# Koukyosyumei/MyZKP

Hardware: AMD Instinct MI355X
Metric: G1 MSM pairs/sec + NTT elems/sec at 2^20 and 2^24; bit-exact vs CPU (higher is better)
Workload: dtype u32x9 (29-bit limbs, 254-bit Montgomery); 1 GPU; KZG commit = BN254 G1 Pippenger MSM of 2^20 (scalar, point) pairs per GPU against a device-resident SRS (commit_kzg, kzg.rs:57-59); 17-bit signed windows (library default at this size), 15 window tables built once at upload; N GPUs = one MSM of N*2^20 pairs (BASELINE configs[2]/[3]); pairs_per_gpu=1048576, seed=332211571536, window_bits=17

## Files before the change

### myzkp_amd/csrc/mzk_msm.hip

```cpp
#include <stdlib.h>
#include <type_traits>
#include "mzk_common.h"
#include "mzk_ec.h"
#include "mzk_coop.h"
#include "mzk_row.h"
#include "mzk_glv.h"
#include "mzk_affine_wave.h"

namespace mzk {

static const MsmKnobs& msm_knobs() {
  static const MsmKnobs k = [] {
    const MsmKnobs d;
    return MsmKnobs{tune_int("MZK_GLV_C", d.glv_c), tune_int("MZK_SMALL_SCAN", d.small_scan), tune_int("MZK_SCAN_MAX_LOG", d.scan_max_log),
                    tune_int("MZK_ACC_PREFETCH", d.acc_prefetch), tune_int("MZK_ACC_SEG", d.acc_seg), tune_int("MZK_COARSE_LOG_20", d.coarse_log_20),
                    tune_int("MZK_COARSE_LOG_17", d.coarse_log_17), tune_int("MZK_PER_FINE", d.per_fine), tune_int("MZK_SORT_SCAN_FREE", d.sort_scan_free),
                    tune_int("MZK_COMBINE_WIDE_MIN_LOG", d.combine_wide_min_log)};
  }();
  return k;
}

int msm_generic_window_bits(size_t n) { return choose_shape_glv(n ? n : 1, msm_knobs().glv_c).c; }

__device__ __forceinline__ void load_words8(const u32* __restrict__ g, u32* w) {
  const uint4* p4 = reinterpret_cast<const uint4*>(g);
  uint4 a = p4[0], b = p4[1];
  w[0] = a.x; w[1] = a.y; w[2] = a.z; w[3] = a.w; w[4] = b.x; w[5] = b.y; w[6] = b.z; w[7] = b.w;
}
__device__ __forceinline__ void store_words8(u32* __restrict__ g, const u32* w) {
  uint4* p4 = reinterpret_cast<uint4*>(g);
  p4[0] = make_uint4(w[0], w[1], w[2], w[3]);
  p4[1] = make_uint4(w[4], w[5], w[6], w[7]);
}
__device__ __forceinline__ Xyzz xyzz_gload(const u32* __restrict__ g, size_t idx) {
  u32 w[32];
#pragma unroll
  for (int q = 0; q < 4; q++) load_words8(g + idx * 32 + 8 * q, w + 8 * q);
  return xyzz_load(w);
}
__device__ __forceinline__ void xyzz_gstore(u32* __restrict__ g, size_t idx, const Xyzz& p) {
  u32 w[32];
  xyzz_store(p, w);
#pragma unroll
  for (int q = 0; q < 4; q++) store_words8(g + idx * 32 + 8 * q, w + 8 * q);
}

static_assert(SLOT_WORDS == 4 * FqParams::L, "a slot is the four raw coordinates");
__device__ __forceinline__ void xyzz_gstore_raw(u32* __restrict__ g, size_t idx, const Xyzz& p) {
  u32 w[SLOT_WORDS];
  const bool inf = xyzz_is_inf(p);
#pragma unroll
  for (int i = 0; i < FqParams::L; i++) {
    w[i] = inf ? 0u : p.X.l[i]; w[9 + i] = inf ? 0u : p.Y.l[i]; w[18 + i] = inf ? 0u : p.ZZ.l[i]; w[27 + i] = inf ? 0u : p.ZZZ.l[i];
  }
  uint4* p4 = reinterpret_cast<uint4*>(g + idx * SLOT_WORDS);
#pragma unroll
  for (int q = 0; q < SLOT_WORDS / 4; q++) p4[q] = make_uint4(w[4 * q], w[4 * q + 1], w[4 * q + 2], w[4 * q + 3]);
}
__device__ __forceinline__ Xyzz xyzz_gload_raw(const u32* __restrict__ g, size_t idx) {
  u32 w[SLOT_WORDS];
  const uint4* p4 = reinterpret_cast<const uint4*>(g + idx * SLOT_WORDS);
#pragma unroll
  for (int q = 0; q < SLOT_WORDS / 4; q++) { const uint4 v = p4[q]; w[4 * q] = v.x; w[4 * q + 1] = v.y; w[4 * q + 2] = v.z; w[4 * q + 3] = v.w; }
  Xyzz p;
#pragma unroll
  for (int i = 0; i < FqParams::L; i++) { p.X.l[i] = w[i]; p.Y.l[i] = w[9 + i]; p.ZZ.l[i] = w[18 + i]; p.ZZZ.l[i] = w[27 + i]; }
  return p;
}
__device__ __forceinline__ Xyzz xyzz_gload_raw_quad(const u32* __restrict__ g, size_t idx, int lane) {
  Fq mine;
  const u32* src = g + idx * SLOT_WORDS + 9 * lane;
#pragma unroll
  for (int i = 0; i < FqParams::L; i++) mine.l[i] = src[i];
  Xyzz p;
  p.X = quad_bcast<0>(mine);
  p.Y = quad_bcast<1>(mine);
  p.ZZ = quad_bcast<2>(mine);
  p.ZZZ = quad_bcast<3>(mine);
  return p;
}

__global__ void k_prepare_points(const u32* __restrict__ in, u32* __restrict__ out, size_t n, u32* __restrict__ phi_out) {
  const size_t i = (size_t)blockIdx.x * blockDim.x + threadIdx.x;
  if (i >= n) return;
  u32 w[16];
  load_words8(in + i * 16, w);
  load_words8(in + i * 16 + 8, w + 8);
  Affine a;
  const bool inf = affine_words_is_inf(w);
  if (!inf) {
    a = affine_load_plain(w);
    affine_store_mont(a, w);
  }
  store_words8(out + i * 16, w);
  store_words8(out + i * 16 + 8, w + 8);
  if (phi_out) {
    if (!inf) {
      Fq beta;
// ... 614 lines not shown
#pragma unroll
    for (int k = 0; k < STAGE_PER_LANE; k++) rk[k] = (chunk + tid + k * SORT2_THREADS < cend) ? counter_inc_agg(cnt, REC::fine(r[k], fmask, fb)) : 0u;
    __syncthreads();
    u32 local = 0;
    for (int q = 0; q < per; q++) { const int f = tid * per + q; if (f < F) local += cnt[f]; }
    u32 run = block_excl_scan<SORT2_THREADS>(local, scan, nullptr);
    for (int q = 0; q < per; q++) { const int f = tid * per + q; if (f < F) { lpre[f] = run; run += cnt[f]; } }
    __syncthreads();
#pragma unroll
    for (int k = 0; k < STAGE_PER_LANE; k++) {
      if (chunk + tid + k * SORT2_THREADS < cend) {
        const u32 fk = REC::fine(r[k], fmask, fb);
        const u32 pos = lpre[fk] + rk[k];
        spay[pos] = REC::payload(r[k], fb);
        skey[pos] = (unsigned short)fk;
      }
    }
    __syncthreads();
    const u32 m = cend - chunk;
    for (u32 j = tid; j < m; j += SORT2_THREADS) {
      const u32 f = skey[j];
      entries[gbase[f] + (j - lpre[f])] = spay[j];
    }
    __syncthreads();
    for (int f = tid; f < F; f += SORT2_THREADS) gbase[f] += cnt[f];
    __syncthreads();
  }
}

__global__ __launch_bounds__(256) void k_scan_local(const u32* __restrict__ in, u32* __restrict__ out, u32* __restrict__ block_sums, size_t n) {
  __shared__ u32 sh[256];
  const size_t base = (size_t)blockIdx.x * SCAN_BLOCK + (size_t)threadIdx.x * SCAN_ITEMS;
  u32 v[SCAN_ITEMS], sum = 0;
#pragma unroll
  for (int k = 0; k < SCAN_ITEMS; k++) {
    v[k] = (base + k < n) ? in[base + k] : 0u;
    sum += v[k];
  }
  u32 block_total;
  u32 excl = block_excl_scan<256>(sum, sh, &block_total);
  if (threadIdx.x == 255) block_sums[blockIdx.x] = block_total;
#pragma unroll
  for (int k = 0; k < SCAN_ITEMS; k++) {
    if (base + k < n) out[base + k] = excl;
    excl += v[k];
  }
}
__global__ __launch_bounds__(256) void k_scan_finish(u32* __restrict__ offsets, const u32* __restrict__ block_sums, size_t nblocks, size_t n) {
  __shared__ u32 part[4];
  static_assert(SCAN_BLOCK % 256 == 0, "one block index per workgroup");
  const size_t i = (size_t)blockIdx.x * blockDim.x + threadIdx.x;
  const size_t first = (size_t)blockIdx.x * blockDim.x;
  const bool total_wg = first >= n;
  const size_t blk = total_wg ? nblocks : first / SCAN_BLOCK;
  u32 acc = 0;
  for (size_t j = threadIdx.x; j < blk; j += 256) acc += block_sums[j];
#pragma unroll
  for (int d = 32; d >= 1; d >>= 1) acc += (u32)__shfl_xor((int)acc, d, 64);
  if ((threadIdx.x & 63) == 0) part[threadIdx.x >> 6] = acc;
  __syncthreads();
  const u32 pre = part[0] + part[1] + part[2] + part[3];
  if (total_wg) { if (threadIdx.x == 0) offsets[n] = pre; }
  else if (i < n) offsets[i] = offsets[i] + pre;
}

__global__ __launch_bounds__(256) void k_scan_add(u32* __restrict__ offsets, const u32* __restrict__ prefix, size_t nblocks, size_t n) {
  const size_t i = (size_t)blockIdx.x * blockDim.x + threadIdx.x;
  if (i < n) offsets[i] += prefix[i / SCAN_BLOCK];
  else if (i == n) offsets[n] = prefix[nblocks];
}
static int launch_exclusive_scan(const u32* in, u32* out, size_t n, u32* scratch, hipStream_t s) {
  const size_t sb = (n + SCAN_BLOCK - 1) / SCAN_BLOCK;
  hipLaunchKernelGGL(k_scan_local, dim3((unsigned)sb), dim3(256), 0, s, in, out, scratch, n);
  if (sb <= SCAN_DIRECT_BLOCKS) {
    hipLaunchKernelGGL(k_scan_finish, dim3((unsigned)((n + 255) / 256 + 1)), dim3(256), 0, s, out, (const u32*)scratch, sb, n);
  } else {
    MZK_TRY(launch_exclusive_scan((const u32*)scratch, scratch, sb, scratch + sb + 2, s));
    hipLaunchKernelGGL(k_scan_add, dim3((unsigned)(n / 256 + 1)), dim3(256), 0, s, out, (const u32*)scratch, sb, n);
  }
  MZK_HIP(hipGetLastError());
  return MZK_OK;
}

constexpr u32 MANY_SENTINEL = 0xffffffffu;
constexpr u32 SEG_MIN = 8;
__device__ __forceinline__ u32 segment_length(u32 seg_host, u32 t_max, u32 total_entries) {
  if (t_max == 0) return seg_host;
  const u32 v = (total_entries + t_max - 1) / t_max;
  return v < SEG_MIN ? SEG_MIN : v;
}
template <bool PREFETCH, bool SENT = false>
__global__ __launch_bounds__(256) void k_seg_accumulate(const u32* __restrict__ points_mont, const u32* __restrict__ offsets,
                                                         const u32* __restrict__ entries, u32* __restrict__ slots, size_t nbuckets,
                                                         u32 seg_host, u32 t_max) {
  const size_t t = (size_t)blockIdx.x * blockDim.x + threadIdx.x;
  const u32 total_entries = offsets[nbuckets];
  const u32 seg = segment_length(seg_host, t_max, total_entries);
  const u64 e0w = (u64)t * seg;
  if (e0w >= total_entries) return;
  const u32 e0 = (u32)e0w;
  const u32 e1 = (e0w + seg < total_entries) ? e0 + seg : total_entries;
  size_t lo = 0, hi = nbuckets;
  while (hi - lo > 1) {
    const size_t mid = (lo + hi) >> 1;
    if (offsets[mid] <= e0) lo = mid; else hi = mid;
  }
  size_t b = lo;
  u32 bend = offsets[b + 1];
  Xyzz acc = xyzz_inf();
  u32 ent_next = entries[e0];
  u32 wn[16];
  if (PREFETCH) {
    const size_t idx = ent_next & 0x7fffffffu;
    load_words8(points_mont + idx * 16, wn);
    load_words8(points_mont + idx * 16 + 8, wn + 8);
  }
  for (u32 e = e0; e < e1; e++) {
    const u32 ent = ent_next;
    u32 w[16];
    if (PREFETCH) {
#pragma unroll
      for (int k = 0; k < 16; k++) w[k] = wn[k];
    } else {
      const size_t idx = (SENT && ent == MANY_SENTINEL) ? 0 : (ent & 0x7fffffffu);
      load_words8(points_mont + idx * 16, w);
      load_words8(points_mont + idx * 16 + 8, w + 8);
    }
    if (e + 1 < e1) {
      ent_next = entries[e + 1];
      if (PREFETCH) {
        const size_t idx = ent_next & 0x7fffffffu;
        load_words8(points_mont + idx * 16, wn);
        load_words8(points_mont + idx * 16 + 8, wn + 8);
      }
    }
    if (e >= bend) {
      xyzz_gstore_raw(slots, t + b, acc);
      acc = xyzz_inf();
      do { b++; bend = offsets[b + 1]; } while (e >= bend);
    }
    if (affine_words_is_inf(w)) continue;
    if (SENT && ent == MANY_SENTINEL) continue;
    acc = xyzz_madd_signed_with<FeAsm>(acc, affine_load_mont(w), (ent >> 31) != 0);
  }
  xyzz_gstore_raw(slots, t + b, acc);
}
constexpr u32 HEAVY_SLOTS_SORT1 = 16;
__device__ __forceinline__ u32 bucket_end(const u32* __restrict__ offsets, const u32* __restrict__ tails, int lg_nb, size_t b) {
  if (tails && (b & (((size_t)1 << lg_nb) - 1)) == (((size_t)1 << lg_nb) - 1)) return tails[b >> lg_nb];
  return offsets[b + 1];
}
__device__ __forceinline__ bool defer_heavy(size_t b, size_t s0, size_t s1, u32 o1, u32* __restrict__ heavy, bool leader, u32 threshold = HEAVY_SLOTS) {
  if (s1 - s0 + 1 <= threshold) return false;
  if (leader) { const u32 i = atomicAdd(&heavy[0], 1u); heavy[HEAVY_HDR + 2 * i] = (u32)b; heavy[HEAVY_HDR + 2 * i + 1] = o1; }
  return true;
}
__global__ __launch_bounds__(128) void k_seg_combine_wide(const u32* __restrict__ slots, const u32* __restrict__ offsets,
                                                           u32* __restrict__ buckets, size_t nbuckets, u32 seg_host, u32* __restrict__ heavy, u32 t_max) {
  const size_t b = (size_t)blockIdx.x * blockDim.x + threadIdx.x;
  if (b >= nbuckets) return;
  const u32 seg = segment_length(seg_host, t_max, offsets[nbuckets]);
  if (b == 0) heavy[1] = seg;
  const u32 o0 = offsets[b], o1 = offsets[b + 1];
  Xyzz acc = xyzz_inf();
  if (o1 > o0) {
    const size_t s0 = (size_t)(o0 / seg) + b, s1 = (size_t)((o1 - 1) / seg) + b;
    if (defer_heavy(b, s0, s1, o1, heavy, true)) return;
    for (size_t sl = s0; sl <= s1; sl++) acc = xyzz_add_with<FeAsm>(acc, xyzz_gload_raw(slots, sl));
  }
  xyzz_gstore(buckets, b, acc);
}
__global__ __launch_bounds__(128) void k_seg_combine(const u32* __restrict__ slots, const u32* __restrict__ offsets, u32* __restrict__ buckets,
                                                      size_t nbuckets, u32 seg_host, u32* __restrict__ heavy, const u32* __restrict__ tails, int lg_nb, u32 t_max) {
  const size_t tid = (size_t)blockIdx.x * blockDim.x + threadIdx.x;
  const size_t b = tid / 4;
  const int lane = (int)(tid & 3);
  if (b >= nbuckets) return;
  const u32 seg = segment_length(seg_host, t_max, offsets[nbuckets]);
  if (tid == 0) heavy[1] = seg;
  const u32 o0 = offsets[b], o1 = bucket_end(offsets, tails, lg_nb, b);
  Xyzz acc = xyzz_inf();
  if (o1 > o0) {
    const size_t s0 = (size_t)(o0 / seg) + b, s1 = (size_t)((o1 - 1) / seg) + b;
    if (defer_heavy(b, s0, s1, o1, heavy, lane == 0, tails ? HEAVY_SLOTS_SORT1 : HEAVY_SLOTS)) return;
    acc = xyzz_gload_raw_quad(slots, s0, lane);
    for (size_t sl = s0 + 1; sl <= s1; sl++) acc = xyzz_add_quad(acc, xyzz_gload_raw_quad(slots, sl, lane), lane);
  }
  xyzz_gstore_quad(buckets, b, acc, lane);
}
constexpr int HEAVY_THREADS = 256;
constexpr int HEAVY_QUADS = HEAVY_THREADS / 4;
__device__ __forceinline__ void heavy_tree(u32* sh, const Xyzz& acc, int quad, int lane) {
  xyzz_gstore_quad(sh, quad, acc, lane);
  __syncthreads();
  for (int off = HEAVY_QUADS / 2; off >= 1; off >>= 1) {
    if (quad < off) {
      const Xyzz x = xyzz_gload_quad(sh, quad, lane), y = xyzz_gload_quad(sh, quad + off, lane);
      xyzz_gstore_quad(sh, quad, xyzz_add_quad(x, y, lane), lane);
    }
    __syncthreads();
  }
}
__global__ __launch_bounds__(HEAVY_THREADS) void k_seg_combine_heavy(const u32* __restrict__ slots, const u32* __restrict__ offsets,
                                                                      u32* __restrict__ buckets, u32* __restrict__ heavy, size_t max_heavy) {
  __shared__ __attribute__((aligned(16))) u32 sh[HEAVY_QUADS * 32];
  __shared__ u32 last_arrival;
  const u32 count = heavy[0];
  if (count == 0) return;
  const u32 seg = heavy[1];
  const int lane = threadIdx.x & 3, quad = threadIdx.x >> 2;
  const u32* list = heavy + HEAVY_HDR;
  if (2 * count > gridDim.x) {
    for (u32 h = blockIdx.x; h < count; h += gridDim.x) {
      const size_t b = list[2 * h];
      const u32 o0 = offsets[b], o1 = list[2 * h + 1];
      const size_t s0 = (size_t)(o0 / seg) + b, s1 = (size_t)((o1 - 1) / seg) + b;
      Xyzz acc = xyzz_inf();
      for (size_t sl = s0 + quad; sl <= s1; sl += HEAVY_QUADS) acc = xyzz_add_quad(acc, xyzz_gload_raw_quad(slots, sl, lane), lane);
      heavy_tree(sh, acc, quad, lane);
      if (quad == 0) xyzz_gstore_quad(buckets, b, xyzz_gload_quad(sh, 0, lane), lane);
      __syncthreads();
    }
    return;
  }
  const u32 G = gridDim.x / count;
  const u32 h = blockIdx.x / G, part = blockIdx.x % G;
  if (h >= count) return;
  u32* scratch = heavy + heavy_list_words(max_heavy);
// ... 398 lines not shown
      *slots = nullptr, *wghist = nullptr, *wsum = nullptr;
  const struct { WsSlot slot; size_t bytes; u32** p; size_t words; } req[] = {
      {WS_MSM_POINTS, P.ws.points, &pm, 0}, {WS_MSM_COUNTS, P.ws.counts, &counts, 0}, {WS_MSM_OFFSETS, P.ws.offsets, &offsets, P.NBtot + 1},
      {WS_MSM_CURSOR, P.ws.cursor, &ranks, 0}, {WS_MSM_ENTRIES, P.ws.entries, &entries, P.alloc.E}, {WS_MSM_SCAN, P.ws.scan, &scan, 0},
      {WS_MSM_BUCKETS, P.ws.buckets, &buckets, P.NB * 32}, {WS_MSM_SLOTS, P.ws.slots, &slots, P.slot_region_words},
      {WS_MSM_WGHIST, P.ws.wghist, &wghist, 0}, {WS_MSM_OUT, P.ws.out, &wsum, 0}};
  for (const auto& r : req)
    if (r.bytes) { MZK_TRY(ws_get(r.slot, r.bytes, (void**)r.p)); *r.p += (cc ? cc->k : 0) * r.words; }
  const u32* pts = (pm ? pm : (const u32*)d_points) + i0 * 16;
  bool prepared = false;
  auto prepare = [&]() -> int {
    if (prepared) return MZK_OK;
    prepared = true;
    if (points_ready) MZK_TRY((*points_ready)());
    if (!pm) return MZK_OK;
    prof_begin(s, MZK_PH_MSM_PREPARE);
    MZK_TRY(msm_prepare_points((const u32*)d_points + i0 * 16, n, pm + i0 * 16, pm + (n_shape + i0) * 16, s));
    prof_end(s, MZK_PH_MSM_PREPARE);
    return MZK_OK;
  };
  if (P.path == MsmPath::SmallScan) {
    MZK_TRY(prepare());
    prof_begin(s, MZK_PH_MSM_ACCUMULATE);
#define MZK_SCAN_CASE(C) case C: hipLaunchKernelGGL((k_small_accumulate_scan<256, C>), dim3((unsigned)P.NB), dim3(256), 0, s, (const u32*)d_scalars, n, P.L.table_stride, pts, buckets); break;
    switch (P.L.c) { MZK_SCAN_CASE(8) MZK_SCAN_CASE(10) MZK_SCAN_CASE(11) MZK_SCAN_CASE(12) MZK_SCAN_CASE(13) }
#undef MZK_SCAN_CASE
    prof_end(s, MZK_PH_MSM_ACCUMULATE);
  } else if (P.path == MsmPath::SmallSort) {
    MZK_TRY(prepare());
    prof_begin(s, MZK_PH_MSM_SORT);
    hipLaunchKernelGGL(k_small_sort, dim3(1), dim3(SMALL_SORT_THREADS), (P.NB + SMALL_SORT_THREADS) * 4, s, (const u32*)d_scalars, n, P.L, (int)P.NB, offsets, entries);
    prof_end(s, MZK_PH_MSM_SORT);
    prof_begin(s, MZK_PH_MSM_ACCUMULATE);
    if (P.small_wide)
      hipLaunchKernelGGL(k_small_accumulate<256>, dim3((unsigned)P.NB), dim3(256), 0, s, pts, (const u32*)offsets, (const u32*)entries, buckets);
    else
      hipLaunchKernelGGL(k_small_accumulate<64>, dim3((unsigned)P.NB), dim3(64), 0, s, pts, (const u32*)offsets, (const u32*)entries, buckets);
    prof_end(s, MZK_PH_MSM_ACCUMULATE);
  } else {
    u32* heavy = slots + P.nslots * SLOT_WORDS;
    prof_begin(s, MZK_PH_MSM_SORT);
    MZK_HIP(hipMemsetAsync(heavy, 0, (size_t)HEAVY_HDR * 4, s));
    if (P.path == MsmPath::TwoLevel) {
      u32* finehist = wghist + P.alloc.n_coarse + 1;
      const SortBufs sb{(const u32*)d_scalars, wghist, ranks, finehist, scan + scan_scratch_words(P.alloc.n_coarse) + 2, offsets, entries,
                        P.coarse_free ? heavy + SORT_CTR_AT : nullptr, P.coarse_free ? heavy + SORT_CTR_AT + SORT_CTR_BINS : nullptr,
                        P.coarse_free ? finehist + P.alloc.n_fine + 1 : nullptr, P.fine_free ? counts : nullptr, P.fine_free ? counts + P.NBtot : nullptr};
#define MZK_CCOUNT(C, CLOG) hipLaunchKernelGGL((k_coarse_count<C, CLOG>), dim3(P.nwg), dim3(SORT2_THREADS), 0, s, (const u32*)d_scalars, n, P.L, P.key_shift, wghist, \
                                               P.nwg, sb.bin_tot, sb.bucket_tot, P.fine_free ? 2 * P.NBtot : (size_t)0)
      if (P.coarse_c == 20 && P.cl == 10) MZK_CCOUNT(20, 10);
      else if (P.coarse_c == 17 && P.cl == 9) MZK_CCOUNT(17, 9);
      else if (P.cl == 10) MZK_CCOUNT(0, 10);
      else if (P.coarse_c == 20) MZK_CCOUNT(20, COARSE_LOG);
      else if (P.coarse_c == 17) MZK_CCOUNT(17, COARSE_LOG);
      else if (P.coarse_c == 16) MZK_CCOUNT(16, COARSE_LOG);
      else MZK_CCOUNT(0, COARSE_LOG);
#undef MZK_CCOUNT
      if (!P.coarse_free) MZK_TRY(launch_exclusive_scan((const u32*)wghist, wghist, P.own.n_coarse, scan, s));
      MZK_TRY(P.compact ? sort_records<Rec4>(P, sb, s) : sort_records<Rec8>(P, sb, s));
    } else if (P.path == MsmPath::LdsOnePass) {
      const size_t lds = P.NB * 4;
      bool& lds_attr_set = ctx().attr_done[ATTR_DIGITS_LDS];
      if (!lds_attr_set) {
        MZK_HIP(hipFuncSetAttribute((const void*)k_digits_count_lds, hipFuncAttributeMaxDynamicSharedMemorySize, 160 * 1024));
        MZK_HIP(hipFuncSetAttribute((const void*)k_digits_scatter_lds, hipFuncAttributeMaxDynamicSharedMemorySize, 160 * 1024));
        lds_attr_set = true;
      }
      hipLaunchKernelGGL(k_digits_count_lds, dim3(P.nwg), dim3(LDS_SORT_THREADS), lds, s, (const u32*)d_scalars, n, P.per_wg, P.L, wghist, ranks);
      hipLaunchKernelGGL(k_wg_hist_prefix, dim3((unsigned)((P.NB + 255) / 256)), dim3(256), 0, s, wghist, P.nwg, (int)P.NB, counts);
      MZK_TRY(launch_exclusive_scan((const u32*)counts, offsets, P.NB, scan, s));
      hipLaunchKernelGGL(k_digits_scatter_lds, dim3(P.nwg), dim3(LDS_SORT_THREADS), lds, s, (const u32*)d_scalars, n, P.per_wg, P.L, (const u32*)offsets,
                         (const u32*)wghist, (const u32*)ranks, entries);
    } else {
      const unsigned nblk = (unsigned)((n + 255) / 256);
      MZK_HIP(hipMemsetAsync(counts, 0, P.NB * 4, s));
      hipLaunchKernelGGL(k_digits_count, dim3(nblk), dim3(256), 0, s, (const u32*)d_scalars, n, P.L, counts, ranks);
      MZK_TRY(launch_exclusive_scan((const u32*)counts, offsets, P.NB, scan, s));
      hipLaunchKernelGGL(k_digits_scatter, dim3(nblk), dim3(256), 0, s, (const u32*)d_scalars, n, P.L, offsets, ranks, entries);
    }
    MZK_HIP(hipGetLastError());
    prof_end(s, MZK_PH_MSM_SORT);
    MZK_TRY(prepare());
    prof_begin(s, MZK_PH_MSM_ACCUMULATE);
#ifdef MZK_TUNING
    if (P.prefetch)
      hipLaunchKernelGGL(k_seg_accumulate<true>, dim3((unsigned)((P.T + 255) / 256)), dim3(256), 0, s, pts, offsets, entries, slots, P.NB, P.seg, P.t_max);
    else
#endif
      hipLaunchKernelGGL(k_seg_accumulate<false>, dim3((unsigned)((P.T + 255) / 256)), dim3(256), 0, s, pts, offsets, entries, slots, P.NB, P.seg, P.t_max);
    prof_end(s, MZK_PH_MSM_ACCUMULATE);
    prof_begin(s, MZK_PH_MSM_SEG_COMBINE);
    if (P.combine_wide)
      hipLaunchKernelGGL(k_seg_combine_wide, dim3((unsigned)((P.NB + 127) / 128)), dim3(128), 0, s, slots, offsets, buckets, P.NB, P.seg, heavy, P.t_max);
    else
      hipLaunchKernelGGL(k_seg_combine, dim3((unsigned)((4 * P.NB + 127) / 128)), dim3(128), 0, s, slots, offsets, buckets, P.NB, P.seg, heavy, (const u32*)nullptr, 0, P.t_max);
    hipLaunchKernelGGL(k_seg_combine_heavy, dim3(HEAVY_GRID), dim3(HEAVY_THREADS), 0, s, (const u32*)slots, (const u32*)offsets, buckets, heavy, P.max_heavy);
    MZK_HIP(hipGetLastError());
    prof_end(s, MZK_PH_MSM_SEG_COMBINE);
    if (cc) return MZK_OK;
  }
  MZK_TRY(reduce_bucket_sets(buckets, P.lgB, P.red_windows, P.one_set, P.horner_c, wsum, (u32*)d_out, out_partial_xyzz, s));
  MZK_HIP(hipGetLastError());
  return MZK_OK;
}

__global__ __launch_bounds__(128) void k_fold_bucket_sets(u32* __restrict__ buckets, size_t NB, int K) {
  const size_t b = (size_t)blockIdx.x * blockDim.x + threadIdx.x;
  if (b >= NB) return;
  Xyzz acc = xyzz_gload(buckets, b);
  for (int k = 1; k < K; k++) acc = xyzz_add_with<FeAsm>(acc, xyzz_gload(buckets, (size_t)k * NB + b));
  xyzz_gstore(buckets, b, acc);
}
bool msm_chunkable(size_t n_total, int point_kind, size_t table_stride) { return msm_chunkable(n_total, point_kind, table_stride, msm_knobs()); }
int msm_chunked_impl(const MsmChunk* chunks, int K, const void* d_points, size_t n_total, int point_kind, size_t table_stride, void* d_out,
                     bool out_partial_xyzz, hipStream_t s, const std::function<int(int)>* before_chunk) {
  if (!chunks || K < 1 || K > 8 || !d_out || !d_points) { set_error("msm_chunked: bad argument"); return MZK_E_ARG; }
  size_t n_alloc = 0, covered = 0;
  for (int k = 0; k < K; k++) {
    if (chunks[k].i0 != covered) { set_error("msm_chunked: chunks must be consecutive"); return MZK_E_ARG; }
    covered += chunks[k].n;
    n_alloc = chunks[k].n > n_alloc ? chunks[k].n : n_alloc;
  }
  if (covered != n_total || !msm_chunkable(n_total, point_kind, table_stride)) { set_error("msm_chunked: chunks do not cover a chunkable problem"); return MZK_E_ARG; }
  for (int k = 0; k < K; k++) {
    if (before_chunk) MZK_TRY((*before_chunk)(k));
    if (chunks[k].ready) MZK_HIP(hipStreamWaitEvent(s, chunks[k].ready, 0));
    const MsmChunkCtx cc{k, K, chunks[k].i0, n_total, n_alloc};
    MZK_TRY(msm_dev_impl(chunks[k].d_scalars, d_points, chunks[k].n, point_kind, table_stride, d_out, out_partial_xyzz, s, nullptr, &cc));
  }
  const MsmPlan P = msm_plan(n_alloc, n_total, n_alloc, point_kind, table_stride, ctx().num_cu, K, msm_knobs());
  u32 *buckets, *wsum;
  MZK_TRY(ws_get(WS_MSM_BUCKETS, P.ws.buckets, (void**)&buckets));
  MZK_TRY(ws_get(WS_MSM_OUT, (size_t)MAX_WINDOWS * 128, (void**)&wsum));
  if (K > 1) {
    prof_begin(s, MZK_PH_MSM_SEG_COMBINE);
    hipLaunchKernelGGL(k_fold_bucket_sets, dim3((unsigned)((P.NB + 127) / 128)), dim3(128), 0, s, buckets, P.NB, K);
    MZK_HIP(hipGetLastError());
    prof_end(s, MZK_PH_MSM_SEG_COMBINE);
  }
  MZK_TRY(reduce_bucket_sets(buckets, P.lgB, P.red_windows, P.one_set, P.horner_c, wsum, (u32*)d_out, out_partial_xyzz, s));
  MZK_HIP(hipGetLastError());
  return MZK_OK;
}

constexpr int MANY_CHUNK = 1024;
constexpr int MANY_THREADS = 256;
constexpr int MANY_PER_LANE = MANY_CHUNK / MANY_THREADS;
template <int C>
__global__ __launch_bounds__(MANY_THREADS) void k_many_count(const u32* __restrict__ scalars, size_t n, size_t stride_words, int nch, u32* __restrict__ cnt) {
  constexpr int NB = 1 << (C - 1);
  __shared__ u32 hist[NB];
  const size_t j = blockIdx.x / (unsigned)nch;
  const int ch = (int)(blockIdx.x % (unsigned)nch);
  for (int b = threadIdx.x; b < NB; b += MANY_THREADS) hist[b] = 0;
  __syncthreads();
  const u32* sc = scalars + j * stride_words;
  const size_t lo = (size_t)ch * MANY_CHUNK;
  const size_t hi = (lo + MANY_CHUNK < n) ? lo + MANY_CHUNK : n;
  u32 w[MANY_PER_LANE][8];
#pragma unroll
  for (int k = 0; k < MANY_PER_LANE; k++) {
    const size_t i = lo + threadIdx.x + (size_t)k * MANY_THREADS;
    if (i < hi) load_scalar_canonical(sc, i, w[k]);
  }
#pragma unroll
  for (int k = 0; k < MANY_PER_LANE; k++) {
    const size_t i = lo + threadIdx.x + (size_t)k * MANY_THREADS;
    if (i < hi) walk_digits_merged<C>(w[k], 0, i, [&](int, u32 key, u32) { counter_inc_agg(hist, key); });
  }
  __syncthreads();
  for (int b = threadIdx.x; b < NB; b += MANY_THREADS) cnt[(j * NB + b) * (size_t)nch + ch] = hist[b];
}
// ... 75 lines not shown
    if (i < n) walk_digits_merged<C>(w[k], table_stride, i, [&](int, u32 key, u32 payload) { stage[counter_inc_agg(hist, key)] = payload; });
  }
  __syncthreads();
  for (u32 e = tid; e < cap; e += SORT1_THREADS) entries[base + e] = (e < total) ? stage[e] : MANY_SENTINEL;
}

bool msm_many_supported(int window_bits) { return window_bits == 8 || (window_bits >= 10 && window_bits <= 13); }

int msm_many_dev_impl(const void* d_scalars, size_t n, size_t stride_elems, size_t count, const void* d_tables, int c, size_t table_stride, void* d_out,
                      hipStream_t s) {
  if (count == 0) return MZK_OK;
  if (!d_out || ((!d_scalars || !d_tables) && n)) { set_error("msm_many: null pointer"); return MZK_E_ARG; }
  if (!msm_many_supported(c)) { set_error("msm_many: window width %d has no grid-batched path", c); return MZK_E_ARG; }
  if (n == 0) {
    MZK_HIP(hipMemsetAsync(d_out, 0, count * 64, s));
    return MZK_OK;
  }
  const int nwin = msm_table_windows(c), lgB = c - 1;
  const size_t NB = (size_t)1 << lgB;
  if ((size_t)nwin * table_stride > ((size_t)1 << 31)) { set_error("msm_many: table rows exceed the 31-bit point references"); return MZK_E_ARG; }
  const int nch = (int)((n + MANY_CHUNK - 1) / MANY_CHUNK);
  size_t per_pass = ((size_t)1 << 21) / NB;
  const size_t by_coefs = (((size_t)1 << 22) + n - 1) / n;
  if (by_coefs < per_pass) per_pass = by_coefs;
  if (per_pass < 1) per_pass = 1;
  for (size_t first = 0; first < count; first += per_pass) {
    const size_t cnt = (count - first < per_pass) ? count - first : per_pass;
    const u32* sc = (const u32*)d_scalars + first * stride_elems * 8;
    u32* out = (u32*)d_out + first * 16;
    const size_t NBtot = cnt * NB, ncnt = NBtot * (size_t)nch;
    const size_t E_max = cnt * n * (size_t)nwin;
    const size_t resident_lanes = (size_t)ctx().num_cu * 4 * 4 * 64;
    size_t seg_sz = (E_max + resident_lanes - 1) / resident_lanes;
    if (seg_sz < 16) seg_sz = 16;
    const u32 seg = (u32)seg_sz;
    const size_t T = (E_max + seg_sz - 1) / seg_sz;
    const size_t nslots = T + NBtot + 1;
    const size_t max_heavy = (T + NBtot) / HEAVY_SLOTS_SORT1 + 1;
    const size_t heavy_words = heavy_total_words(max_heavy);
    u32 *offs, *compact, *entries, *scan_tmp, *buckets, *slots;
    MZK_TRY(ws_get(WS_MSM_COUNTS, (ncnt + 1) * 4, (void**)&offs));
    MZK_TRY(ws_get(WS_MSM_ENTRIES, E_max * 4, (void**)&entries));
    MZK_TRY(ws_get(WS_MSM_SCAN, scan_scratch_words(ncnt) * 4, (void**)&scan_tmp));
    MZK_TRY(ws_get(WS_MSM_BUCKETS, NBtot * 128, (void**)&buckets));
    MZK_TRY(ws_get(WS_MSM_SLOTS, nslots * SLOT_WORDS * 4 + heavy_words * 4, (void**)&slots));
    compact = offs;
    u32* tails = nullptr;
    if (nch > 1) MZK_TRY(ws_get(WS_MSM_OFFSETS, (NBtot + 1) * 4, (void**)&compact));
    else MZK_TRY(ws_get(WS_MSM_OFFSETS, cnt * 4, (void**)&tails));
    u32* heavy = slots + nslots * SLOT_WORDS;
    prof_begin(s, MZK_PH_MSM_SORT);
    MZK_HIP(hipMemsetAsync(heavy, 0, (size_t)HEAVY_HDR * 4, s));
    const unsigned nwg = (unsigned)(cnt * (size_t)nch);
    const bool one_kernel_sort = nch == 1;
    if (one_kernel_sort) {
      bool& done = ctx().attr_done[ATTR_MANY_SORT1];
      if (!done) {
        MZK_HIP(hipFuncSetAttribute((const void*)k_many_sort1<8>, hipFuncAttributeMaxDynamicSharedMemorySize, 140 * 1024));
        MZK_HIP(hipFuncSetAttribute((const void*)k_many_sort1<10>, hipFuncAttributeMaxDynamicSharedMemorySize, 140 * 1024));
        MZK_HIP(hipFuncSetAttribute((const void*)k_many_sort1<11>, hipFuncAttributeMaxDynamicSharedMemorySize, 140 * 1024));
        MZK_HIP(hipFuncSetAttribute((const void*)k_many_sort1<12>, hipFuncAttributeMaxDynamicSharedMemorySize, 140 * 1024));
        MZK_HIP(hipFuncSetAttribute((const void*)k_many_sort1<13>, hipFuncAttributeMaxDynamicSharedMemorySize, 140 * 1024));
        done = true;
      }
    }
#define MZK_MANY_CASE(C) case C:                                                                                                                    \
      if (one_kernel_sort) {                                                                                                                         \
        hipLaunchKernelGGL((k_many_sort1<C>), dim3(nwg), dim3(SORT1_THREADS), n * (size_t)nwin * 4, s, sc, n, stride_elems * 8, table_stride,       \
                           (u32)(n * (size_t)nwin), offs, cnt, entries, tails);                                                                           \
        break;                                                                                                                                       \
      }                                                                                                                                              \
      hipLaunchKernelGGL((k_many_count<C>), dim3(nwg), dim3(MANY_THREADS), 0, s, sc, n, stride_elems * 8, nch, offs);                                \
      MZK_TRY(launch_exclusive_scan((const u32*)offs, offs, ncnt, scan_tmp, s));                                                                     \
      hipLaunchKernelGGL((k_many_scatter<C>), dim3(nwg), dim3(MANY_THREADS), 0, s, sc, n, stride_elems * 8, nch, table_stride, (const u32*)offs,     \
                         nch > 1 ? compact : (u32*)nullptr, NBtot, entries);                                                                         \
      break;
    switch (c) { MZK_MANY_CASE(8) MZK_MANY_CASE(10) MZK_MANY_CASE(11) MZK_MANY_CASE(12) MZK_MANY_CASE(13) }
#undef MZK_MANY_CASE
    MZK_HIP(hipGetLastError());
    prof_end(s, MZK_PH_MSM_SORT);
    prof_begin(s, MZK_PH_MSM_ACCUMULATE);
    const u32 t_max = one_kernel_sort ? 0u : (u32)T;
    if (one_kernel_sort)
      hipLaunchKernelGGL((k_seg_accumulate<false, true>), dim3((unsigned)((T + 255) / 256)), dim3(256), 0, s, (const u32*)d_tables, (const u32*)compact, (const u32*)entries,
                         slots, NBtot, seg, t_max);
    else
      hipLaunchKernelGGL(k_seg_accumulate<false>, dim3((unsigned)((T + 255) / 256)), dim3(256), 0, s, (const u32*)d_tables, (const u32*)compact, (const u32*)entries,
                         slots, NBtot, seg, t_max);
    prof_end(s, MZK_PH_MSM_ACCUMULATE);
    prof_begin(s, MZK_PH_MSM_SEG_COMBINE);
    const unsigned cgrid = (unsigned)((4 * NBtot + 127) / 128);
    hipLaunchKernelGGL(k_seg_combine, dim3(cgrid), dim3(128), 0, s, slots, (const u32*)compact, buckets, NBtot, seg, heavy, (const u32*)tails, lgB, t_max);
    hipLaunchKernelGGL(k_seg_combine_heavy, dim3(HEAVY_GRID), dim3(HEAVY_THREADS), 0, s, (const u32*)slots, (const u32*)compact, buckets, heavy, max_heavy);
    MZK_HIP(hipGetLastError());
    prof_end(s, MZK_PH_MSM_SEG_COMBINE);
    prof_begin(s, MZK_PH_MSM_REDUCE);
    int t_start = 0;
    MZK_TRY(launch_halving_steps(buckets, lgB, (int)cnt, row_tail_max_ops(), &t_start, s));
    MZK_TRY(launch_reduce_tail_row(buckets, lgB, t_start, (int)cnt, out, 1, s));
    MZK_HIP(hipGetLastError());
    prof_end(s, MZK_PH_MSM_REDUCE);
  }
  return MZK_OK;
}

constexpr int DIRECT_THREADS = 256;
size_t msm_direct_bytes(size_t n, int c) { return (size_t)msm_table_windows(c) * n * ((size_t)1 << (c - 1)) * 64; }
__global__ __launch_bounds__(64) void k_direct_chain(const u32* __restrict__ rows_mont, size_t rows, int M, u32* __restrict__ out_xyzz) {
  const size_t r = (size_t)blockIdx.x * blockDim.x + threadIdx.x;
  if (r >= rows) return;
  u32 w[16];
  load_words8(rows_mont + r * 16, w);
  load_words8(rows_mont + r * 16 + 8, w + 8);
  const bool inf = affine_words_is_inf(w);
  const Affine a = affine_load_mont(w);
  Xyzz acc = xyzz_inf();
  for (int m = 0; m < M; m++) {
    if (!inf) acc = xyzz_madd_signed_with<FeCpp>(acc, a, false);
    xyzz_gstore(out_xyzz, r * (size_t)M + m, acc);
  }
}
int msm_build_direct(const void* d_points_mont, size_t n, int c, void* d_direct, hipStream_t s) {
  if (n == 0) return MZK_OK;
  const int nwin = msm_table_windows(c), M = 1 << (c - 1);
  const size_t rows = (size_t)nwin * n;
  u32 *tables, *tmp;
  MZK_TRY(ws_get(WS_MISC_C, rows * 64, (void**)&tables));
  MZK_TRY(msm_build_tables(d_points_mont, n, tables, c, s));
  size_t slice = ((size_t)1 << 21) / (size_t)M;
  if (slice < 64) slice = 64;
  if (slice > rows) slice = rows;
  MZK_TRY(ws_get(WS_MISC_D, slice * (size_t)M * 128, (void**)&tmp));
  for (size_t r0 = 0; r0 < rows; r0 += slice) {
    const size_t cnt = (rows - r0 < slice) ? rows - r0 : slice;
    hipLaunchKernelGGL(k_direct_chain, dim3((unsigned)((cnt + 63) / 64)), dim3(64), 0, s, (const u32*)tables + r0 * 16, cnt, M, tmp);
    MZK_HIP(hipGetLastError());
    MZK_TRY(xyzz_batch_to_affine(tmp, cnt * (size_t)M, (u32*)d_direct + r0 * (size_t)M * 16, true, s));
  }
  return MZK_OK;
}
template <int C>
__device__ __forceinline__ bool direct_item(const u32* __restrict__ sc, size_t t, size_t table_stride, const u32* __restrict__ direct, const u32** rec, bool* neg) {
  constexpr int NWIN = 254 / C + 1;
  constexpr u32 HALF = 1u << (C - 1), MASKC = (1u << C) - 1u;
  const size_t i = t / NWIN;
  const int win = (int)(t - i * NWIN);
  u32 w[8], tw[10];
  load_scalar_canonical(sc, i, w);
  u64 cy = 0;
#pragma unroll
  for (int k = 0; k < 8; k++) { cy += (u64)w[k] + digit_bias_word(C, k); tw[k] = (u32)cy; cy >>= 32; }
  tw[8] = (u32)cy + digit_bias_word(C, 8);
  tw[9] = 0;
  const int bit = win * C, k = bit >> 5, sft = bit & 31;
  u32 lo = tw[0], hi = tw[1];
#pragma unroll
  for (int q = 1; q < 9; q++) { lo = (k == q) ? tw[q] : lo; hi = (k == q) ? tw[q + 1] : hi; }
  const u32 v = (u32)((((u64)hi << 32) | lo) >> sft) & MASKC;
  if (v == HALF - 1u) return false;
  *neg = v < HALF - 1u;
  const u32 mag = *neg ? (HALF - 1u) - v : v - (HALF - 1u);
  *rec = direct + (((size_t)win * table_stride + i) * HALF + (mag - 1u)) * 16;
  return true;
}
template <int C>
__global__ __launch_bounds__(DIRECT_THREADS) void k_direct_accumulate(const u32* __restrict__ scalars, size_t n, size_t stride_words, int parts, size_t table_stride,
                                                                       const u32* __restrict__ direct, u32* __restrict__ slots) {
// ... 224 lines not shown
```

### myzkp_amd/csrc/mzk_msm_plan.h

```cpp
#pragma once
#include <stddef.h>
#include <stdint.h>
#include <stdio.h>
#include "../../include/mzk.h"

namespace mzk {

enum { MSM_PTS_PLAIN = 0, MSM_PTS_MONT = 1, MSM_PTS_TABLES = 2 };
static inline int msm_table_windows(int c) { return 254 / c + 1; }
static inline int msm_table_rows(int c, int sets) { return 254 / (c * sets) + 1; }

constexpr int SCALAR_BITS = 254;
constexpr int MAX_WINDOWS = 32;
constexpr int GLV_MAG_BITS = 126;
constexpr int SLOT_WORDS = 36;

struct DigitLayout {
  int c, nwin, merged;
  int sets;
  size_t table_stride;
  int glv;
  size_t phi_offset;
};

struct MsmShape { int c, nwin, lgB; size_t nbuckets; };
static MsmShape choose_shape_glv(size_t n, int force_c = 0) {
  int lg = 0;
  while (((size_t)1 << lg) < 2 * n) lg++;
  int c = lg - 3;
  if (c < 8) c = 8;
  if (c > 16) c = 16;
  if (c == 15) c = 16;
  if (n >= ((size_t)3 << 21)) c = 19;
  if (force_c > 0) c = force_c;
  for (; c > 8; c--) {
    const int nw = GLV_MAG_BITS / c + 1;
    if (GLV_MAG_BITS - c * (nw - 1) >= 5) break;
  }
  MsmShape s;
  s.c = c;
  s.nwin = GLV_MAG_BITS / c + 1;
  s.lgB = c - 1;
  s.nbuckets = (size_t)s.nwin << s.lgB;
  return s;
}

#ifndef MZK_COARSE_LOG
#define MZK_COARSE_LOG 8
#endif
constexpr int COARSE_LOG = MZK_COARSE_LOG;
constexpr int COARSE_PER_WG = 4096;
constexpr int FINE_MAX = 8192;
constexpr int STAGE_F_MAX = 2048;
constexpr size_t SMALL_MAX_N = 4097;
constexpr size_t SMALL_MAX_BUCKETS = 8192;
constexpr int SCAN_ITEMS = 8;
constexpr int SCAN_BLOCK = 256 * SCAN_ITEMS;
constexpr size_t SCAN_DIRECT_BLOCKS = 2048;
static inline size_t scan_scratch_words(size_t n) {
  const size_t sb = (n + SCAN_BLOCK - 1) / SCAN_BLOCK;
  return sb + 2 + (sb > SCAN_DIRECT_BLOCKS ? scan_scratch_words(sb) : 0);
}
constexpr uint32_t HEAVY_SLOTS = 32;
constexpr int HEAVY_GRID = 512;
constexpr int SORT_CTR_BINS = 1024;
constexpr int SORT_CTR_AT = 2 + HEAVY_GRID;
constexpr int HEAVY_HDR = SORT_CTR_AT + 2 * SORT_CTR_BINS;
constexpr size_t heavy_list_words(size_t max_heavy) { return (HEAVY_HDR + 2 * max_heavy + 2 + 3) & ~(size_t)3; }
constexpr size_t heavy_total_words(size_t max_heavy) { return heavy_list_words(max_heavy) + (size_t)HEAVY_GRID * 32 + 8; }

struct MsmKnobs {
  int glv_c = 0;
  int small_scan = 1;
  int scan_max_log = 14;
  int acc_prefetch = -1;
  int acc_seg = 0;
  int coarse_log_20 = 10;
  int coarse_log_17 = 9;
  int per_fine = 0;
  int sort_scan_free = 3;
  int combine_wide_min_log = 17;
};

enum class MsmPath { SmallScan, SmallSort, TwoLevel, LdsOnePass, Atomic };
struct MsmWsBytes { size_t points, counts, offsets, cursor, entries, buckets, scan, slots, wghist, out; };
struct MsmSizing { size_t E, T, n_coarse, n_fine; };

struct MsmPlan {
  int err = MZK_OK;
  char msg[192] = {};
  size_t n = 0;
  DigitLayout L{};
  int lgB = 0, red_windows = 0, horner_c = 0;
  size_t NB = 0, NBtot = 0;
  bool one_set = false, small_wide = false;
  MsmPath path = MsmPath::SmallSort;
  int cl = 0, F = 0, fb = 0, key_shift = 0, S = 0, nwg = 0;
  uint32_t fine_mask = 0, slice_cap = 0;
  unsigned fine_wgs = 0;
  size_t per_wg = 0;
  bool compact = false, coarse_free = false, fine_free = false, scatter_staged = false;
  int coarse_c = 0;
  uint32_t seg = 0, t_max = 0;
  size_t T = 0, nslots = 0, max_heavy = 0, slot_region_words = 0;
  bool prefetch = false, combine_wide = false;
  MsmSizing own{}, alloc{};
  MsmWsBytes ws{}, ws_used{};
  MsmPlan& fail(const char* fmt, size_t a = 0, size_t b = 0, size_t c = 0) { err = MZK_E_ARG; snprintf(msg, sizeof msg, fmt, a, b, c); return *this; }
};

static inline size_t msm_slot_region_words(size_t T, size_t NB) {
  return ((T + NB + 1) * SLOT_WORDS + heavy_total_words((T + NB) / HEAVY_SLOTS + 1) + 3) & ~(size_t)3;
}
static inline MsmPlan& msm_sized(MsmPlan& P, size_t regions) {
  for (int u = 0; u < 2; u++) {
    const MsmSizing& z = u ? P.own : P.alloc;
    MsmWsBytes& w = u ? P.ws_used : P.ws;
    w.points = P.ws.points, w.out = P.ws.out;
    w.offsets = regions * (P.NBtot + 1) * 4;
    w.entries = regions * z.E * 4;
    w.buckets = regions * P.NB * 128;
    if (P.path == MsmPath::SmallScan || P.path == MsmPath::SmallSort) continue;
    const bool two = P.path == MsmPath::TwoLevel;
    w.counts = 2 * P.NBtot * 4;
    w.cursor = z.E * (two ? 8 : 4);
    w.slots = regions * msm_slot_region_words(z.T, P.NB) * 4;
    w.wghist = two ? (z.n_coarse + 1 + z.n_fine + 1 + ((size_t)1 << P.cl) + 1) * 4 : P.path == MsmPath::LdsOnePass ? (size_t)P.nwg * P.NB * 4 : 0;
    w.scan = two ? (scan_scratch_words(z.n_coarse) + scan_scratch_words(z.n_fine) + 4) * 4 : scan_scratch_words(P.NB) * 4;
  }
  return P;
}

static inline MsmPlan msm_plan(size_t n, size_t n_shape, size_t n_alloc, int point_kind, size_t table_stride, int num_cu, int chunks,
                               const MsmKnobs& kn) {
  MsmPlan P;
  P.n = n;
  if (n > ((size_t)1 << 27)) return P.fail("msm: n > 2^27 not supported");
  const int kind = point_kind & 0xff, table_c = (point_kind >> 8) & 0xff, table_sets = (point_kind >> 16) & 0xff;
  DigitLayout& L = P.L;
  L.merged = kind == MSM_PTS_TABLES;
  L.sets = (L.merged && table_sets) ? table_sets : 1;
  L.table_stride = table_stride;
  L.glv = !L.merged;
  L.phi_offset = kind == MSM_PTS_PLAIN ? n_shape : table_stride;
  const MsmShape sh = choose_shape_glv(n_shape, kn.glv_c);
  L.c = L.merged ? (table_c ? table_c : 16) : sh.c;
  L.nwin = L.merged ? msm_table_windows(L.c) : sh.nwin;
  P.NB = L.merged ? (size_t)L.sets << (L.c - 1) : sh.nbuckets;
  P.lgB = L.c - 1, P.red_windows = L.merged ? L.sets : L.nwin;
  P.one_set = L.merged && L.sets == 1, P.horner_c = P.one_set ? 0 : L.c;
  const size_t windows_per_pair = L.glv ? 2 * L.nwin : L.nwin, regions = chunks ? chunks : 1;
  const size_t E_max = P.own.E = n * windows_per_pair, E_alloc = P.alloc.E = n_alloc * windows_per_pair;
  P.ws.points = kind == MSM_PTS_PLAIN ? 2 * n_shape * 64 : 0;
  P.ws.out = chunks ? 0 : (size_t)MAX_WINDOWS * 128;
  P.NBtot = P.NB;
  if (L.glv && (P.NB & (P.NB - 1)) != 0 && L.c >= 17) { P.NBtot = 1; while (P.NBtot < P.NB) P.NBtot <<= 1; }

  const bool scan_ok = P.one_set && kn.small_scan != 0 && n <= ((size_t)1 << kn.scan_max_log) && (L.c == 8 || (L.c >= 10 && L.c <= 13));
  if (!chunks && (scan_ok || n < (L.merged ? SMALL_MAX_N : SMALL_MAX_N - 1)) && P.NB <= SMALL_MAX_BUCKETS) {
    P.path = scan_ok ? MsmPath::SmallScan : MsmPath::SmallSort;
    P.small_wide = E_max / P.NB > 64;
    return msm_sized(P, 1);
  }
  const size_t ref_max = L.merged ? (size_t)msm_table_rows(L.c, L.sets) * table_stride : L.phi_offset + n;
  if (ref_max > ((size_t)1 << 31) || E_max >= ((size_t)1 << 32))
    return P.fail("msm: %zu pairs x %zu windows (table stride %zu) exceed the 31-bit point references / 32-bit entry offsets", n, (size_t)L.nwin, table_stride);

  P.prefetch = kn.acc_prefetch > 0;
  const size_t resident_lanes = (size_t)num_cu * 4 * (P.prefetch ? 3 : 4) * 64;
  size_t seg = (E_max + resident_lanes - 1) / resident_lanes;
  seg = kn.acc_seg > 0 ? (size_t)kn.acc_seg : seg < 16 ? 16 : seg;
  P.seg = (uint32_t)seg;
  P.T = P.own.T = (E_max + seg - 1) / seg;
  P.t_max = kn.acc_seg > 0 ? 0u : (uint32_t)P.T;
  P.nslots = P.T + P.NB + 1;
  P.max_heavy = (P.T + P.NB) / HEAVY_SLOTS + 1;
  P.combine_wide = P.NB >= ((size_t)1 << kn.combine_wide_min_log);
  const size_t T_seg = E_alloc / (kn.acc_seg > 0 ? (size_t)kn.acc_seg : 16) + 1;
  P.alloc.T = !chunks ? P.T : kn.acc_seg > 0 ? T_seg : (resident_lanes + 1 < T_seg ? resident_lanes + 1 : T_seg);
  P.slot_region_words = msm_slot_region_words(P.alloc.T, P.NB);

  const bool plain_merged = L.merged && L.sets == 1;
  P.cl = (plain_merged && L.c == 20 && kn.coarse_log_20 == 10) ? 10 : COARSE_LOG;
  if (plain_merged && L.c == 17 && kn.coarse_log_17 == 9 && COARSE_LOG == 8 && ref_max > ((size_t)1 << (31 - 8)) && ref_max <= ((size_t)1 << (31 - 7)))
    P.cl = 9;
  if (L.glv && P.NBtot > ((size_t)STAGE_F_MAX << COARSE_LOG)) P.cl = 10;
  const size_t cbins = (size_t)1 << P.cl;
  const bool two_level = (P.NBtot & (P.NBtot - 1)) == 0 && P.NBtot >= 4096 && (P.NBtot / cbins) <= (size_t)FINE_MAX &&
                         (n >= 4096 || (L.merged && P.NBtot > ((size_t)1 << 15)));
  if (chunks && !two_level) return P.fail("msm: chunk mode needs the two-level sort (layout %zu bits, %zu buckets)", (size_t)L.c, P.NB);
  P.path = two_level ? MsmPath::TwoLevel : L.merged ? MsmPath::LdsOnePass : MsmPath::Atomic;
  if (P.path == MsmPath::LdsOnePass) {
    const size_t nwg = (n + 4095) / 4096;
    P.nwg = nwg < 1 ? 1 : nwg > (size_t)num_cu ? num_cu : (int)nwg;
    P.per_wg = (n + P.nwg - 1) / P.nwg;
  }
  if (!two_level) return msm_sized(P, regions);
  while (((size_t)1 << P.key_shift) < P.NBtot) P.key_shift++;
  P.key_shift -= P.cl;
  P.F = (int)(P.NBtot / cbins);
  P.fine_mask = (uint32_t)P.F - 1u;
  while ((1 << P.fb) < P.F) P.fb++;
  P.nwg = (int)((n + COARSE_PER_WG - 1) / COARSE_PER_WG);
  const size_t per_fine = kn.per_fine > 0 ? (size_t)kn.per_fine : (P.F >= 4096 ? 131072 : P.F >= 2048 ? 65536 : (L.glv ? 16384 : 32768));
  const size_t S = (E_max / cbins + per_fine - 1) / per_fine;
  P.S = S < 2 ? 2 : S > 64 ? 64 : (int)S;
  const size_t slice_nom = (E_max + cbins * (size_t)P.S - 1) / (cbins * (size_t)P.S);
  P.slice_cap = (uint32_t)(slice_nom + slice_nom / 2 + 1);
  P.fine_wgs = (unsigned)(cbins * (size_t)P.S + (E_max + P.slice_cap - 1) / P.slice_cap + 1);
  P.own.n_coarse = cbins * P.nwg;
  P.own.n_fine = (size_t)P.F * P.fine_wgs;
  const size_t slice_nom_a = (E_alloc + cbins * (size_t)64 - 1) / (cbins * (size_t)64);
  P.alloc.n_coarse = chunks ? cbins * ((n_alloc + COARSE_PER_WG - 1) / COARSE_PER_WG) : P.own.n_coarse;
  P.alloc.n_fine = chunks ? (size_t)P.F * (cbins * 64 + (E_alloc + slice_nom_a) / (slice_nom_a + slice_nom_a / 2 + 1) + 2) : P.own.n_fine;
  P.compact = ref_max <= ((size_t)1 << (31 - P.fb));
  P.coarse_free = (kn.sort_scan_free & 1) != 0 && cbins <= (size_t)SORT_CTR_BINS;
  P.fine_free = (kn.sort_scan_free & 2) != 0 && P.F <= STAGE_F_MAX;
  P.coarse_c = (plain_merged && (L.c == 16 || L.c == 17 || L.c == 20)) ? L.c : 0;
  P.scatter_staged = P.coarse_c != 0;
  return msm_sized(P, regions);
}

static inline bool msm_chunkable(size_t n_total, int point_kind, size_t table_stride, const MsmKnobs& kn) {
  if (n_total < ((size_t)1 << 18)) return false;
  const MsmPlan P = msm_plan(n_total, n_total, n_total, point_kind, table_stride, 256, 1, kn);
  return P.err == MZK_OK && P.L.sets == 1 && P.path == MsmPath::TwoLevel;
}

}
```

Before: 755.3 million pairs/s.

## Software-pipeline point loads in segmented accumulate and use k-ary bucket search

Rewrites the segmented bucket-accumulate kernel around a shared walker that prefetches the next entry two ahead and issues the next point-row load before the current add. It also precomputes the following bucket end, and replaces the binary bucket search with a 16/32-ary search that batches offset loads. Launch bounds now request 3 waves per SIMD, and the segment sizing is fixed to match, removing the old tuning-only prefetch path. The intent is to hide global-memory latency of point fetches behind the EC addition. The cost is more live registers, and the occupancy cap may cause spills.

```diff
diff --git a/myzkp_amd/csrc/mzk_msm.hip b/myzkp_amd/csrc/mzk_msm.hip
--- a/myzkp_amd/csrc/mzk_msm.hip
+++ b/myzkp_amd/csrc/mzk_msm.hip
@@ -13,7 +13,7 @@
   static const MsmKnobs k = [] {
     const MsmKnobs d;
     return MsmKnobs{tune_int("MZK_GLV_C", d.glv_c), tune_int("MZK_SMALL_SCAN", d.small_scan), tune_int("MZK_SCAN_MAX_LOG", d.scan_max_log),
-                    tune_int("MZK_ACC_PREFETCH", d.acc_prefetch), tune_int("MZK_ACC_SEG", d.acc_seg), tune_int("MZK_COARSE_LOG_20", d.coarse_log_20),
+                    tune_int("MZK_ACC_SEG", d.acc_seg), tune_int("MZK_COARSE_LOG_20", d.coarse_log_20),
                     tune_int("MZK_COARSE_LOG_17", d.coarse_log_17), tune_int("MZK_PER_FINE", d.per_fine), tune_int("MZK_SORT_SCAN_FREE", d.sort_scan_free),
                     tune_int("MZK_COMBINE_WIDE_MIN_LOG", d.combine_wide_min_log)};
   }();
@@ -794,68 +794,45 @@
   return MZK_OK;
 }
 
-constexpr u32 MANY_SENTINEL = 0xffffffffu;
 constexpr u32 SEG_MIN = 8;
 __device__ __forceinline__ u32 segment_length(u32 seg_host, u32 t_max, u32 total_entries) {
   if (t_max == 0) return seg_host;
   const u32 v = (total_entries + t_max - 1) / t_max;
   return v < SEG_MIN ? SEG_MIN : v;
 }
-template <bool PREFETCH, bool SENT = false>
-__global__ __launch_bounds__(256) void k_seg_accumulate(const u32* __restrict__ points_mont, const u32* __restrict__ offsets,
+template <bool SENT = false>
+__global__ __launch_bounds__(256, 3) void k_seg_accumulate(const u32* __restrict__ points_mont, const u32* __restrict__ offsets,
                                                          const u32* __restrict__ entries, u32* __restrict__ slots, size_t nbuckets,
                                                          u32 seg_host, u32 t_max) {
   const size_t t = (size_t)blockIdx.x * blockDim.x + threadIdx.x;
   const u32 total_entries = offsets[nbuckets];
-  const u32 seg = segment_length(seg_host, t_max, total_entries);
-  const u64 e0w = (u64)t * seg;
-  if (e0w >= total_entries) return;
-  const u32 e0 = (u32)e0w;
-  const u32 e1 = (e0w + seg < total_entries) ? e0 + seg : total_entries;
-  size_t lo = 0, hi = nbuckets;
-  while (hi - lo > 1) {
-    const size_t mid = (lo + hi) >> 1;
-    if (offsets[mid] <= e0) lo = mid; else hi = mid;
-  }
-  size_t b = lo;
-  u32 bend = offsets[b + 1];
+  u32 e0, e1;
+  if (!seg_span(t, segment_length(seg_host, t_max, total_entries), total_entries, &e0, &e1)) return;
+  const auto offset_at = [&](size_t b) __attribute__((always_inline)) { return offsets[b]; };
   Xyzz acc = xyzz_inf();
-  u32 ent_next = entries[e0];
-  u32 wn[16];
-  if (PREFETCH) {
-    const size_t idx = ent_next & 0x7fffffffu;
-    load_words8(points_mont + idx * 16, wn);
-    load_words8(points_mont + idx * 16 + 8, wn + 8);
-  }
-  for (u32 e = e0; e < e1; e++) {
-    const u32 ent = ent_next;
-    u32 w[16];
-    if (PREFETCH) {
-#pragma unroll
-      for (int k = 0; k < 16; k++) w[k] = wn[k];
-    } else {
-      const size_t idx = (SENT && ent == MANY_SENTINEL) ? 0 : (ent & 0x7fffffffu);
-      load_words8(points_mont + idx * 16, w);
-      load_words8(points_mont + idx * 16 + 8, w + 8);
-    }
-    if (e + 1 < e1) {
-      ent_next = entries[e + 1];
-      if (PREFETCH) {
-        const size_t idx = ent_next & 0x7fffffffu;
-        load_words8(points_mont + idx * 16, wn);
-        load_words8(points_mont + idx * 16 + 8, wn + 8);
-      }
-    }
-    if (e >= bend) {
-      xyzz_gstore_raw(slots, t + b, acc);
-      acc = xyzz_inf();
-      do { b++; bend = offsets[b + 1]; } while (e >= bend);
-    }
-    if (affine_words_is_inf(w)) continue;
-    if (SENT && ent == MANY_SENTINEL) continue;
-    acc = xyzz_madd_signed_with<FeAsm>(acc, affine_load_mont(w), (ent >> 31) != 0);
-  }
-  xyzz_gstore_raw(slots, t + b, acc);
+  u32 w[16];
+  Affine pt;
+  bool skip = false;
+  seg_walk<SENT>(
+      e0, e1, seg_first_bucket(offset_at, nbuckets, e0), nbuckets, [&](u32 e) __attribute__((always_inline)) { return entries[e]; }, offset_at,
+      [&](u32 ref) __attribute__((always_inline)) {
+        const size_t idx = ref & 0x7fffffffu;
+        load_words8(points_mont + idx * 16, w);
+        load_words8(points_mont + idx * 16 + 8, w + 8);
+      },
+      [&](u32 ent) __attribute__((always_inline)) {
+#pragma unroll
+        for (int k = 0; k < 16; k++) asm volatile("" : "+v"(w[k]));
+        skip = affine_words_is_inf(w) || (SENT && ent == MANY_SENTINEL);
+        pt = affine_load_mont(w);
+      },
+      [&](size_t b) __attribute__((always_inline)) {
+        xyzz_gstore_raw(slots, t + b, acc);
+        acc = xyzz_inf();
+      },
+      [&](u32, u32 ent, size_t) __attribute__((always_inline)) {
+        if (!skip) acc = xyzz_madd_signed_with<FeAsm>(acc, pt, (ent >> 31) != 0);
+      });
 }
 constexpr u32 HEAVY_SLOTS_SORT1 = 16;
 __device__ __forceinline__ u32 bucket_end(const u32* __restrict__ offsets, const u32* __restrict__ tails, int lg_nb, size_t b) {
@@ -1420,12 +1397,7 @@
     prof_end(s, MZK_PH_MSM_SORT);
     MZK_TRY(prepare());
     prof_begin(s, MZK_PH_MSM_ACCUMULATE);
-#ifdef MZK_TUNING
-    if (P.prefetch)
-      hipLaunchKernelGGL(k_seg_accumulate<true>, dim3((unsigned)((P.T + 255) / 256)), dim3(256), 0, s, pts, offsets, entries, slots, P.NB, P.seg, P.t_max);
-    else
-#endif
-      hipLaunchKernelGGL(k_seg_accumulate<false>, dim3((unsigned)((P.T + 255) / 256)), dim3(256), 0, s, pts, offsets, entries, slots, P.NB, P.seg, P.t_max);
+    hipLaunchKernelGGL(k_seg_accumulate<false>, dim3((unsigned)((P.T + 255) / 256)), dim3(256), 0, s, pts, offsets, entries, slots, P.NB, P.seg, P.t_max);
     prof_end(s, MZK_PH_MSM_ACCUMULATE);
     prof_begin(s, MZK_PH_MSM_SEG_COMBINE);
     if (P.combine_wide)
@@ -1667,7 +1639,7 @@
     prof_begin(s, MZK_PH_MSM_ACCUMULATE);
     const u32 t_max = one_kernel_sort ? 0u : (u32)T;
     if (one_kernel_sort)
-      hipLaunchKernelGGL((k_seg_accumulate<false, true>), dim3((unsigned)((T + 255) / 256)), dim3(256), 0, s, (const u32*)d_tables, (const u32*)compact, (const u32*)entries,
+      hipLaunchKernelGGL(k_seg_accumulate<true>, dim3((unsigned)((T + 255) / 256)), dim3(256), 0, s, (const u32*)d_tables, (const u32*)compact, (const u32*)entries,
                          slots, NBtot, seg, t_max);
     else
       hipLaunchKernelGGL(k_seg_accumulate<false>, dim3((unsigned)((T + 255) / 256)), dim3(256), 0, s, (const u32*)d_tables, (const u32*)compact, (const u32*)entries,
diff --git a/myzkp_amd/csrc/mzk_msm_plan.h b/myzkp_amd/csrc/mzk_msm_plan.h
--- a/myzkp_amd/csrc/mzk_msm_plan.h
+++ b/myzkp_amd/csrc/mzk_msm_plan.h
@@ -14,6 +14,7 @@
 constexpr int MAX_WINDOWS = 32;
 constexpr int GLV_MAG_BITS = 126;
 constexpr int SLOT_WORDS = 36;
+constexpr int ACC_RESIDENT_WAVES = 3;
 
 struct DigitLayout {
   int c, nwin, merged;
@@ -73,7 +74,6 @@
   int glv_c = 0;
   int small_scan = 1;
   int scan_max_log = 14;
-  int acc_prefetch = -1;
   int acc_seg = 0;
   int coarse_log_20 = 10;
   int coarse_log_17 = 9;
@@ -103,7 +103,7 @@
   int coarse_c = 0;
   uint32_t seg = 0, t_max = 0;
   size_t T = 0, nslots = 0, max_heavy = 0, slot_region_words = 0;
-  bool prefetch = false, combine_wide = false;
+  bool combine_wide = false;
   MsmSizing own{}, alloc{};
   MsmWsBytes ws{}, ws_used{};
   MsmPlan& fail(const char* fmt, size_t a = 0, size_t b = 0, size_t c = 0) { err = MZK_E_ARG; snprintf(msg, sizeof msg, fmt, a, b, c); return *this; }
@@ -166,8 +166,7 @@
   if (ref_max > ((size_t)1 << 31) || E_max >= ((size_t)1 << 32))
     return P.fail("msm: %zu pairs x %zu windows (table stride %zu) exceed the 31-bit point references / 32-bit entry offsets", n, (size_t)L.nwin, table_stride);
 
-  P.prefetch = kn.acc_prefetch > 0;
-  const size_t resident_lanes = (size_t)num_cu * 4 * (P.prefetch ? 3 : 4) * 64;
+  const size_t resident_lanes = (size_t)num_cu * 4 * ACC_RESIDENT_WAVES * 64;
   size_t seg = (E_max + resident_lanes - 1) / resident_lanes;
   seg = kn.acc_seg > 0 ? (size_t)kn.acc_seg : seg < 16 ? 16 : seg;
   P.seg = (uint32_t)seg;
@@ -221,6 +220,71 @@
   return msm_sized(P, regions);
 }
 
+#if defined(__HIPCC__)
+#define MZK_HD __host__ __device__ __forceinline__
+#else
+#define MZK_HD inline
+#endif
+constexpr uint32_t MANY_SENTINEL = 0xffffffffu;
+
+MZK_HD bool seg_span(uint64_t t, uint32_t seg, uint32_t total, uint32_t* e0, uint32_t* e1) {
+  const uint64_t e0w = t * seg;
+  if (e0w >= total) return false;
+  *e0 = (uint32_t)e0w;
+  *e1 = (e0w + seg < total) ? (uint32_t)e0w + seg : total;
+  return true;
+}
+
+template <int K, class Offset>
+MZK_HD size_t seg_bucket_search(Offset offset_at, size_t nbuckets, uint32_t e) {
+  size_t lo = 0, hi = nbuckets;
+  while (hi - lo > 1) {
+    const size_t step = (hi - lo + K - 1) / K;
+    uint32_t v[K];
+#if defined(__HIPCC__)
+#pragma unroll
+#endif
+    for (int j = 1; j < K; j++) v[j] = offset_at(lo + j * step < hi ? lo + j * step : hi);
+    size_t below = 0;
+#if defined(__HIPCC__)
+#pragma unroll
+#endif
+    for (int j = 1; j < K; j++) below += v[j] <= e ? 1 : 0;
+    lo += below * step;
+    if (lo + step < hi) hi = lo + step;
+  }
+  return lo;
+}
+template <class Offset>
+MZK_HD size_t seg_first_bucket(Offset offset_at, size_t nbuckets, uint32_t e) {
+  return nbuckets <= ((size_t)1 << 20) ? seg_bucket_search<16>(offset_at, nbuckets, e) : seg_bucket_search<32>(offset_at, nbuckets, e);
+}
+
+template <bool SENT, class Entry, class Offset, class IssueRow, class TakeRow, class Flush, class Add>
+MZK_HD void seg_walk(uint32_t e0, uint32_t e1, size_t b, size_t nbuckets, Entry entry_at, Offset offset_at, IssueRow issue_row, TakeRow take_row,
+                     Flush flush, Add add) {
+  const auto row_ref = [](uint32_t ent) { return (SENT && ent == MANY_SENTINEL) ? 0u : ent; };
+  const auto end_after_next = [&](size_t bb) { return offset_at(bb + 2 <= nbuckets ? bb + 2 : nbuckets); };
+  uint32_t ent = entry_at(e0);
+  uint32_t ent1 = entry_at(e1 - e0 > 1 ? e0 + 1 : e0);
+  issue_row(row_ref(ent));
+  uint32_t bend = offset_at(b + 1), bend1 = end_after_next(b);
+  for (uint32_t e = e0; e < e1; e++) {
+    take_row(ent);
+    const uint32_t ent2 = entry_at(e1 - e > 2 ? e + 2 : e1 - 1);
+    issue_row(row_ref(ent1));
+    if (e >= bend) {
+      flush(b);
+      b++, bend = bend1;
+      while (e >= bend) b++, bend = offset_at(b + 1);
+      bend1 = end_after_next(b);
+    }
+    add(e, ent, b);
+    ent = ent1, ent1 = ent2;
+  }
+  flush(b);
+}
+
 static inline bool msm_chunkable(size_t n_total, int point_kind, size_t table_stride, const MsmKnobs& kn) {
   if (n_total < ((size_t)1 << 18)) return false;
   const MsmPlan P = msm_plan(n_total, n_total, n_total, point_kind, table_stride, 256, 1, kn);
```

New measurement: 785.3 million pairs/s (median of 6 runs). 4.0% higher.
